# denix56/SI-Mamba

Hardware: AMD Instinct MI355X
Metric: point-clouds/sec (fwd+bwd) (higher is better)
Workload: dtype f32; 1 GPU; PointMamba classifier train step (FPS+kNN grouping, encoder, spectral SAST ordering, 12 Mamba blocks d=384 at L=1024, head, AdamW), 1024 pts -> 128 patches; global_batch=64, per_gpu_batch=64, npoints=1024, patches=128, mamba_seq_len=1024, parallelism=dp1, communicator_ranks=1, library_gemm=tuned solution table (si_mamba_amd/tuned/gemm_gfx950.csv)

## Files before the change

### include/simamba.h

```cpp
#ifndef SIMAMBA_H_
#define SIMAMBA_H_

#include <stddef.h>

#ifdef __cplusplus
extern "C" {
#endif

#define SIMAMBA_ABI_VERSION 9

#define SIMAMBA_F32  0
#define SIMAMBA_BF16 1

#define SIMAMBA_OK            0
#define SIMAMBA_E_NULLPTR    -1
#define SIMAMBA_E_SHAPE      -2
#define SIMAMBA_E_DTYPE      -3
#define SIMAMBA_E_DSTATE     -4
#define SIMAMBA_E_WIDTH      -5
#define SIMAMBA_E_WORKSPACE  -6
#define SIMAMBA_E_GROUPS     -7
#define SIMAMBA_E_ALIGN      -8
#define SIMAMBA_E_VARIANT    -9
#define SIMAMBA_E_BIAS       -10
// ... 101 lines not shown
                               void* normed, float* mean, float* rstd, int batch, int rows_per_batch,
                               int dim, float eps, int hidden_dtype, int out_dtype, void* stream);
int simamba_add_layer_norm_bwd(const void* dnormed, const float* dresidual_out,
                               const float* residual_out, const float* mean, const float* rstd,
                               const float* weight, const float* rowscale, float* dresidual,
                               void* dhidden, float* dwb_partial, int batch, int rows_per_batch,
                               int dim, int hidden_dtype, int out_dtype, void* stream);

#define SIMAMBA_NORM_RMS 1
int simamba_add_layer_norm_fwd_ex(const void* hidden, const float* residual, const float* rowscale,
                                  const float* weight, const float* bias, float* residual_out,
                                  void* normed, float* mean, float* rstd, int batch, int rows_per_batch,
                                  int dim, float eps, int hidden_dtype, int out_dtype, int flags, void* stream);
int simamba_add_layer_norm_bwd_ex(const void* dnormed, const float* dresidual_out,
                                  const float* residual_out, const float* mean, const float* rstd,
                                  const float* weight, const float* rowscale, float* dresidual,
                                  void* dhidden, float* dwb_partial, int batch, int rows_per_batch,
                                  int dim, int hidden_dtype, int out_dtype, int flags, void* stream);

int simamba_add_layer_norm_check_slots(const int* slots_host, int batch, int compact_batch);
int simamba_add_layer_norm_fwd_slots(const void* hidden, const float* residual, const float* rowscale,
                                     const float* weight, const float* bias, float* residual_out,
                                     void* normed, float* mean, float* rstd, const int* hidden_slot,
                                     int hidden_batch, const int* normed_slot, int normed_batch, int batch,
                                     int rows_per_batch, int dim, float eps, int hidden_dtype, int out_dtype,
                                     int flags, void* stream);
int simamba_add_layer_norm_bwd_slots(const void* dnormed, const float* dresidual_out,
                                     const float* residual_out, const float* mean, const float* rstd,
                                     const float* weight, const float* rowscale, float* dresidual,
                                     void* dhidden, float* dwb_partial, const int* hidden_slot,
                                     int hidden_batch, const int* normed_slot, int normed_batch, int batch,
                                     int rows_per_batch, int dim, int hidden_dtype, int out_dtype, int flags,
                                     void* stream);

int simamba_out_proj_add_ln_fwd(const void* y, const void* w, const float* residual, const float* rowscale,
                                const float* gamma, const float* beta, float* residual_out, void* normed, float* mean,
                                float* rstd, int batch, int K, int L, int C, float eps, int out_dtype, void* stream);
int simamba_out_proj_add_ln_fwd_ex(const void* y, const void* w, const float* residual, const float* rowscale,
                                   const float* gamma, const float* beta, float* residual_out, void* normed,
                                   float* mean, float* rstd, int batch, int K, int L, int C, float eps, int out_dtype,
                                   int flags, void* stream);

int simamba_in_proj_fwd(const void* x, const void* w, void* xz, int batch, int L, int C, int M, int io_dtype,
                        void* stream);

int simamba_bn_relu_grid(long long rows);
int simamba_bn_relu_fwd(const void* x, const float* gterm, int group, const float* weight, const float* bias,
                        float* running_mean, float* running_var, float momentum, float eps, int training,
                        void* y, float* mean, float* invstd, float* partial, long long rows, int C,
                        long long ld, int io_dtype, void* stream);
int simamba_bn_relu_bwd(const void* dy, const void* x, const float* gterm, int group, const float* weight,
                        const float* bias, const float* mean, const float* invstd, void* dx, float* dgterm,
                        int dgroup, float* dweight, float* dbias, float* partial, long long rows, int C,
                        long long ld, int io_dtype, int training, void* stream);
int simamba_bn_stats_local(const void* x, const float* gterm, int group, double* stats, long long stats_ld,
                           float* partial, long long rows, int C, long long ld, int io_dtype, void* stream);
int simamba_bn_stats_merge(const double* stats, int world, float* running_mean, float* running_var, float momentum,
                           float eps, float* mean, float* invstd, double* count, int C, void* stream);
int simamba_bn_relu_apply(const void* x, const float* gterm, int group, const float* weight, const float* bias,
                          const float* mean, const float* invstd, void* y, long long rows, int C, long long ld,
                          int io_dtype, void* stream);
int simamba_bn_relu_bwd_sums(const void* dy, const void* x, const float* gterm, int group, const float* weight,
                             const float* bias, const float* mean, const float* invstd, float* dweight,
                             float* dbias, float* partial, long long rows, int C, long long ld, int io_dtype,
                             void* stream);
int simamba_bn_relu_bwd_dx(const void* dy, const void* x, const float* gterm, int group, const float* weight,
// ... 156 lines not shown
```

### si_mamba_amd/_lib.py

```python
from __future__ import annotations

import ctypes
import os
from ctypes import c_char_p, c_float, c_int, c_longlong, c_size_t, c_uint, c_void_p

_HERE = os.path.dirname(os.path.abspath(__file__))
LIB_PATH = os.path.join(_HERE, "libsimamba_hip.so")

F32, BF16 = 0, 1

SPEC_SYMMETRIC = 0x01
SPEC_SELF_LOOP = 0x02
SPEC_BINARY = 0x04
SPEC_MATRIX_SYM = 0x08
SPEC_SMALLEST = 0x10
SPEC_SIGMA_MEAN = 0x20
SPEC_LARGE_G = 0x40
SPEC_MAX_G = 128
SPEC_MAX_G_LARGE = 512

SCAN_AUTO, SCAN_ROWSCAN, SCAN_LPC2, SCAN_LPC4, SCAN_MIX = 0, 1, 2, 4, 6
CKPT_ROW, CKPT_SEQ = 128, 16
BWD_DETERMINISTIC = 1
NORM_RMS = 1
# ... 38 lines not shown
    "simamba_selective_scan_dt_bwd": (c_int, [_P, _P, _P, _P, _P, _P, _P, _P, _P,
                                              _P, _P, _P, _P, _P, _P, _P, _P,
                                              c_int, c_int, c_int, c_int, c_int, c_int,
                                              _LL, _LL, _LL, _LL, _P]),
    "simamba_selective_scan_dt_bwd_ex": (c_int, [_P, _P, _P, _P, _P, _P, _P, _P, _P,
                                                 _P, _P, _P, _P, _P, _P, _P, _P,
                                                 c_int, c_int, c_int, c_int, c_int, c_int,
                                                 _LL, _LL, _LL, _LL, c_int, _P, _LL, _P]),
    "simamba_xdt_proj_fwd": (c_int, [_P, _P, _P, _P, _P, c_int, c_int, c_int, c_int, c_int, c_int, _LL, _P]),
    "simamba_conv_xdt_proj_fwd": (c_int, [_P, _P, _P, _P, _P, _P, _P, _P, c_int, c_int, c_int, c_int, c_int, c_int, _LL,
                                          _P]),
    "simamba_seq_gather_fwd": (c_int, [_P, _P, _P, c_int, c_int, c_int, c_int, _LL, c_int, _P]),
    "simamba_seq_gather_bwd": (c_int, [_P, _P, _P, c_int, c_int, c_int, c_int, c_int, _LL, c_int, _P]),
    "simamba_causal_conv1d_fwd": (c_int, [_P, _P, _P, _P, c_int, c_int, c_int, c_int, c_int, c_int, _LL, _P]),
    "simamba_causal_conv1d_bwd": (c_int, [_P, _P, _P, _P, _P, _P, _P,
                                          c_int, c_int, c_int, c_int, c_int, c_int, _LL, _LL, _P]),
    "simamba_causal_conv1d_bwd_workspace_floats": (_LL, [c_int, c_int, c_int, c_int, c_int]),
    "simamba_causal_conv1d_bwd_ex": (c_int, [_P, _P, _P, _P, _P, _P, _P,
                                             c_int, c_int, c_int, c_int, c_int, c_int, _LL, _LL, c_int, _P, _LL, _P]),
    "simamba_add_layer_norm_grid": (c_int, [c_int, c_int]),
    "simamba_add_layer_norm_fwd": (c_int, [_P, _P, _P, _P, _P, _P, _P, _P, _P, c_int, c_int, c_int, c_float,
                                           c_int, c_int, _P]),
    "simamba_add_layer_norm_bwd": (c_int, [_P, _P, _P, _P, _P, _P, _P, _P, _P, _P, c_int, c_int, c_int,
                                           c_int, c_int, _P]),
    "simamba_add_layer_norm_fwd_ex": (c_int, [_P, _P, _P, _P, _P, _P, _P, _P, _P, c_int, c_int, c_int, c_float,
                                              c_int, c_int, c_int, _P]),
    "simamba_add_layer_norm_bwd_ex": (c_int, [_P, _P, _P, _P, _P, _P, _P, _P, _P, _P, c_int, c_int, c_int,
                                              c_int, c_int, c_int, _P]),
    "simamba_add_layer_norm_check_slots": (c_int, [_P, c_int, c_int]),
    "simamba_add_layer_norm_fwd_slots": (c_int, [_P, _P, _P, _P, _P, _P, _P, _P, _P, _P, c_int, _P, c_int, c_int, c_int,
                                                 c_int, c_float, c_int, c_int, c_int, _P]),
    "simamba_add_layer_norm_bwd_slots": (c_int, [_P, _P, _P, _P, _P, _P, _P, _P, _P, _P, _P, c_int, _P, c_int, c_int,
                                                 c_int, c_int, c_int, c_int, c_int, _P]),
    "simamba_out_proj_add_ln_fwd": (c_int, [_P, _P, _P, _P, _P, _P, _P, _P, _P, _P, c_int, c_int, c_int, c_int, c_float,
                                            c_int, _P]),
    "simamba_out_proj_add_ln_fwd_ex": (c_int, [_P, _P, _P, _P, _P, _P, _P, _P, _P, _P, c_int, c_int, c_int, c_int,
                                               c_float, c_int, c_int, _P]),
    "simamba_in_proj_fwd": (c_int, [_P, _P, _P, c_int, c_int, c_int, c_int, c_int, _P]),
    "simamba_bn_relu_grid": (c_int, [_LL]),
    "simamba_bn_relu_fwd": (c_int, [_P, _P, c_int, _P, _P, _P, _P, c_float, c_float, c_int, _P, _P, _P, _P, _LL, c_int,
                                    _LL, c_int, _P]),
    "simamba_bn_relu_bwd": (c_int, [_P, _P, _P, c_int, _P, _P, _P, _P, _P, _P, c_int, _P, _P, _P, _LL, c_int, _LL,
                                    c_int, c_int, _P]),
    "simamba_bn_stats_local": (c_int, [_P, _P, c_int, _P, _LL, _P, _LL, c_int, _LL, c_int, _P]),
    "simamba_bn_stats_merge": (c_int, [_P, c_int, _P, _P, c_float, c_float, _P, _P, _P, c_int, _P]),
    "simamba_bn_relu_apply": (c_int, [_P, _P, c_int, _P, _P, _P, _P, _P, _LL, c_int, _LL, c_int, _P]),
    "simamba_bn_relu_bwd_sums": (c_int, [_P, _P, _P, c_int, _P, _P, _P, _P, _P, _P, _P, _LL, c_int, _LL, c_int, _P]),
    "simamba_bn_relu_bwd_dx": (c_int, [_P, _P, _P, c_int, _P, _P, _P, _P, _P, _P, _P, _P, _P, c_int, _LL, c_int, _LL,
                                       c_int, _P]),
    "simamba_group_max_fwd": (c_int, [_P, _P, _P, _LL, c_int, c_int, c_int, _P]),
    "simamba_group_max_bwd": (c_int, [_P, _P, _P, _LL, c_int, c_int, c_int, _P]),
    "simamba_max_linear_bwd_slabs": (c_int, [_LL, c_int]),
    "simamba_max_linear_bwd_dx": (c_int, [_P, _P, _P, _P, _LL, c_int, c_int, c_int, c_int, _P]),
    "simamba_max_linear_bwd_dw": (c_int, [_P, _P, _P, _P, _P, _LL, c_int, c_int, c_int, c_int, _P]),
    "simamba_three_nn": (c_int, [_P, _P, _P, _P, c_int, c_int, c_int, _P]),
    "simamba_three_interpolate_fwd": (c_int, [_P, _P, _P, _P, c_int, c_int, c_int, c_int, c_int, _P]),
    "simamba_three_interpolate_bwd": (c_int, [_P, _P, _P, _P, c_int, c_int, c_int, c_int, c_int, _P]),
    "simamba_gather_sum_scatter": (c_int, [_P, _P, _P, _P, c_int, c_int, c_int, c_int, c_int, c_int, _P]),
    "simamba_chamfer_fwd": (c_int, [_P, _P, _P, _P, _P, _LL, c_int, c_int, _P]),
    "simamba_chamfer_bwd": (c_int, [_P, _P, _P, _P, _P, _P, _LL, c_int, c_int, _P]),
    "simamba_chamfer_large_fwd": (c_int, [_P, _P, _P, _P, _P, _P, _P, _LL, c_int, c_int, _P]),
    "simamba_chamfer_large_bwd": (c_int, [_P, _P, _P, _P, _P, _P, _P, _LL, c_int, c_int, _P]),
    "simamba_chamfer_large_fwd_ex": (c_int, [_P, _P, _P, _P, _P, _P, _P, _LL, c_int, c_int, c_int, _P]),
    "simamba_chamfer_large_bwd_ex": (c_int, [_P, _P, _P, _P, _P, _P, _P, _LL, c_int, c_int, c_int, _P]),
    "simamba_chamfer_ragged_fwd": (c_int, [_P] * 9 + [_LL] + [c_int] * 6 + [_P]),
    "simamba_chamfer_ragged_bwd": (c_int, [_P] * 11 + [_LL] + [c_int] * 6 + [_P]),
# ... 207 lines not shown
    cell, coerce = _fuse_dt, staticmethod(_tristate)


def fuse_dt_enabled(dtype):
    import torch
    return (dtype == torch.bfloat16) if _fuse_dt[0] is None else _fuse_dt[0]


_fuse_out_norm = [True]
_hand_in_proj = [None]


class fuse_out_norm(_Override):
    cell = _fuse_out_norm


def fuse_out_norm_enabled():
    return _fuse_out_norm[0]


_drop_path_compact = [os.environ.get("SIMAMBA_DROP_PATH_COMPACT", "1").strip().lower() not in ("0", "false", "off")]
DROP_PATH_BUCKET = 4
compact_sizes = {}


class drop_path_compact(_Override):
    cell = _drop_path_compact


def drop_path_compact_enabled():
    return _drop_path_compact[0]


_sparse_max_linear = [None]


class sparse_max_linear(_Override):
    cell, coerce = _sparse_max_linear, staticmethod(_tristate)


def sparse_max_linear_enabled(dtype):
    import torch
    return (dtype == torch.float32) if _sparse_max_linear[0] is None else _sparse_max_linear[0]


class hand_in_proj(_Override):
    cell, coerce = _hand_in_proj, staticmethod(_tristate)


def in_proj_hand_enabled(workgroups, dtype=None):
    import torch
    if _hand_in_proj[0] is not None:
        return _hand_in_proj[0]
    return dtype != torch.float32 and workgroups >= IN_PROJ_MIN_WORKGROUPS


IN_PROJ_MIN_WORKGROUPS = 192


def scan_plan_step(batch, dim, seqlen, dstate, dtype, *, softplus=True, has_z=True, act_addr_or=0, a_addr=0,
                   b_addr=0, c_addr=0, z_bs=0, dz_bs=0, bc_strides=(0, 0, 0)):
    lib = load()
    code = dtype_code(dtype)
    step = _scan_ckpt[0] or lib.simamba_scan_ckpt_step(batch, dim, seqlen, dstate, code)
    if step == CKPT_SEQ and not lib.simamba_scan_seq_applicable(
            batch, dim, seqlen, dstate, code, int(bool(softplus)), int(bool(has_z)), act_addr_or, a_addr, b_addr,
# ... 66 lines not shown
```

### si_mamba_amd/block.py

```python
from __future__ import annotations

import math
from functools import partial
from typing import NamedTuple, Optional

import torch
import torch.nn as nn
from torch import Tensor

from . import _lib
from .add_norm import add_layer_norm_fn
from .cross_merge import cross_merge, cross_merge_composed, cross_merge_maps
from .mamba_simple import Mamba
from .out_norm import out_proj_add_ln_fn, out_proj_add_ln_ok
from .rms_norm import RMSNorm
from .spectral import argsort_rows, take

_KERNEL_NORMS = (nn.LayerNorm, RMSNorm)


def _fused_norm(hidden, residual, norm, rowscale=None, out_dtype=None, **compact):
    rms = type(norm) is RMSNorm
    if rms:
        _lib.count("add_rms_norm")
# ... 304 lines not shown
        y = normed = None
        if first == 0:
            l0 = self.layers[0]
            scale = l0.drop_path.rowscale(hidden_states) if isinstance(l0.drop_path, DropPath) else None
            normed, residual = _fused_norm(hidden_states, None, l0.norm, rowscale=scale)
        else:
            y = hidden_states
        n = len(self.layers)
        i = first
        while True:
            if y is not None:
                prev = self.layers[i - 1].mixer
                if i < n:
                    norm, dp = self.layers[i].norm, self.layers[i].drop_path
                    scale = dp.rowscale(y) if isinstance(dp, DropPath) else None
                    out_dtype = y.dtype
                else:
                    norm, scale, out_dtype = self.norm_f, None, self.norm_f.weight.dtype
                if out_proj_add_ln_ok(y, prev.out_proj.weight, prev.d_model):
                    rms = type(norm) is RMSNorm
                    _lib.count("out_proj_add_rms" if rms else "out_proj_add_ln")
                    normed, residual = out_proj_add_ln_fn(y, prev.out_proj.weight, residual, norm.weight, norm.bias,
                                                          norm.eps, rowscale=scale, out_dtype=out_dtype, rms=rms)
                else:
                    hidden = torch.matmul(y.transpose(1, 2), prev.out_proj.weight.t().to(y.dtype))
                    normed, residual = _fused_norm(hidden, residual, norm, rowscale=scale, out_dtype=out_dtype)
                if i == n:
                    return normed
            mixer = self.layers[i].mixer
            y = mixer.forward_xz(mixer.in_proj_xz(normed), A=A_all[i], emit_y=True)
            i += 1

    def forward(self, input_ids, pos, inference_params=None, token_index=None, balanced_index=False, *,
                route=None, drop_plan=None, drop_masks=None):
        if route is None:
            route = self.route(input_ids, token_index.shape[1] if (token_index is not None and balanced_index) else None,
                               inference_params)
        plan = drop_plan
        if plan is None:
            plan = self.draw_drop_plan(input_ids, lead=route.lead, drop_masks=drop_masks, route=route)
        elif route.stack != "compact" or plan.lead != route.lead or plan.batch != input_ids.shape[0]:
            raise ValueError("MixerModel.forward: drop_plan was drawn for another route or batch")
        if plan is not None:
            self._finish_plan(plan, input_ids.device)
            _lib.count("drop_path_compact")
        A_all = self._precompute_A()
        if route.stack == "chain" and drop_masks is not None:
            raise NotImplementedError("MixerModel.forward(drop_masks=...): the fused bf16 chain draws its own factors")
        if route.first_on_tokens:
            hidden_states, residual = self._first_block_on_distinct_tokens(
                input_ids, pos, token_index, A=A_all[0], emit_y=route.stack == "chain",
                keep=None if plan is None else (plan.sel, plan.sizes[0]))
            if plan is not None:
                residual = self._compact_ran(0, hidden_states, residual)
            hidden_states = self.drop_out_in_block(hidden_states)
            first = 1
        else:
            if token_index is not None:
                input_ids, pos = take(input_ids, token_index), take(pos, token_index)
            hidden_states, residual, first = input_ids + pos, None, 0
        if route.stack == "chain":
            return self._chain(first, hidden_states, residual, A_all)
        if plan is not None:
            return self._compact_stack(first, hidden_states, residual, A_all, plan)
        return self._layer_stack(first, hidden_states, residual, A_all, inference_params, drop_masks)

    def _layer_stack(self, first, hidden_states, residual, A_all, inference_params=None, drop_masks=None):
        for i in range(first, len(self.layers)):
            scale = drop_masks[i - 1] if (drop_masks is not None and i > 0) else None
            hidden_states, residual = self.layers[i](hidden_states, residual, inference_params=inference_params,
                                                     A=A_all[i], rowscale=scale)
            hidden_states = self.drop_out_in_block(hidden_states)
        return self._final_norm(hidden_states, residual)

    def _final_norm(self, hidden_states, residual):
        if hidden_states.is_cuda and type(self.norm_f) in _KERNEL_NORMS and hidden_states.dim() == 3:
            return _fused_norm(hidden_states, residual, self.norm_f, out_dtype=self.norm_f.weight.dtype)[0]
        residual = (hidden_states + residual) if residual is not None else hidden_states
        return self.norm_f(residual.to(dtype=self.norm_f.weight.dtype))

    def _compact_ran(self, i, hidden_states, residual):
        if hidden_states is None:
            return _SkippedMixerFn.apply(residual, *self.layers[i].mixer.parameters())
        size = hidden_states.shape[0]
        _lib.compact_sizes[size] = _lib.compact_sizes.get(size, 0) + 1
        return residual

    def _compact_stack(self, first, hidden_states, residual, A_all, plan):
        n, B = len(self.layers), plan.batch
        io = hidden_states.dtype if hidden_states is not None else self.layers[0].mixer.out_proj.weight.dtype
        for i in range(first, n):
            compact = {}
            if i > 0 and plan.sizes[i - 1] < B:
                compact.update(hidden_slot=plan.maps[i - 1], hidden_dtype=io)
            if i < n - 1 and plan.sizes[i] < B:
                compact.update(normed_slot=plan.maps[i], normed_batch=plan.sizes[i])
            hidden_states, residual = self.layers[i](hidden_states, residual, A=A_all[i],
                                                     rowscale=plan.masks[i - 1] if i > 0 else None,
                                                     draw=False, compact=compact)
            residual = self._compact_ran(i, hidden_states, residual)
            if hidden_states is not None:
                io = hidden_states.dtype
        return self._final_norm(hidden_states, residual)


class MixerModel_add(MixerModel):

    composed = False

    def forward(self, input_ids, pos, top_k_eigenvectors, N_k_top_eigenvectors, reverse, inference_params=None, *,
                order=None):
        if not reverse:
            raise ValueError("MixerModel_add: add_after_layer needs reverse=True (with reverse=False the reference "
                             "discards the merge)")
        k = int(N_k_top_eigenvectors)
        if order is None:
            vecs = top_k_eigenvectors[:, :, :k]
            B, G = vecs.shape[:2]
            order = argsort_rows(vecs.transpose(1, 2).reshape(B * k, G)).view(B, k, G)
        if order.shape[1] != k or 2 * k * order.shape[2] != input_ids.shape[1]:
            raise ValueError(f"MixerModel_add: a sequence of {input_ids.shape[1]} tokens is not 2 k G with orders "
                             f"{tuple(order.shape)} and k = {k}")
        maps = None if self.composed else cross_merge_maps(order)
        hidden_states = input_ids + pos
        residual = None
        A_all = self._precompute_A()
        for i, layer in enumerate(self.layers):
            hidden_states, residual = layer(hidden_states, residual, inference_params=inference_params, A=A_all[i])
            hidden_states = self.drop_out_in_block(hidden_states)
            hidden_states = (cross_merge_composed(hidden_states, order) if self.composed
                             else cross_merge(hidden_states, maps))
        return self._final_norm(hidden_states, residual)
```

### si_mamba_amd/point_mamba.py

```python
from __future__ import annotations

from types import SimpleNamespace

import torch
import torch.nn as nn

from . import grouping, spectral
from .block import MixerModel, MixerModel_add
from .add_norm import add_layer_norm_fn
from .encoder_ops import bn_relu_fn, group_max_fn, token_linear, token_linear_group_max


class Group(nn.Module):

    def __init__(self, num_group, group_size):
        super().__init__()
        self.num_group = num_group
        self.group_size = group_size
        self.fps_fn = grouping.sample_farthest_points

    @torch.no_grad()
    def _indices(self, xyz, lengths=None):
        if lengths is not None:
            if not (xyz.is_cuda and xyz.shape[1] <= 8192):
                raise NotImplementedError("Group: lengths are taken by the HIP kernels only (a ROCm device, clouds of "
                                          "up to 8192 points)")
            need = max(self.num_group, self.group_size)
            if not torch.cuda.is_current_stream_capturing():
                shortest = int(lengths.min())
                if shortest < need:
                    raise ValueError(f"Group: the shortest cloud has {shortest} points, every cloud needs at least "
                                     f"{need} (max of num_group = {self.num_group} and group_size = {self.group_size})")
            center, _ = self.fps_fn(xyz, self.num_group, lengths=lengths)
            return center, grouping.knn_group(center, xyz, self.group_size, lengths=lengths)
        center, _ = self.fps_fn(xyz, self.num_group)
        if xyz.is_cuda and xyz.shape[1] <= 8192:
            return center, grouping.knn_group(center, xyz, self.group_size)
        d = torch.cdist(center, xyz)
        nn_idx = d.topk(self.group_size, dim=-1, largest=False, sorted=False)[1]
        return center, nn_idx

    def forward(self, xyz, *, lengths=None):
# ... 88 lines not shown
        self.method = config.method
        self.reverse = config.reverse
        self.k_top_eigenvectors = config.k_top_eigenvectors
        self.smallest = config.smallest
        self.knn_graph = config.knn_graph
        self.symmetric = config.symmetric
        self.self_loop = config.self_loop
        self.alpha = config.alpha
        self.binary = config.binary
        self.matrix = config.matrix
        if self.method not in ("SAST", "HLT", "MAMBA"):
            raise NotImplementedError(f"ordering method {self.method!r}: SAST (:868), HLT (:1054) and MAMBA (:850) "
                                      "are built; the wavelet / RL research branches are out of scope")
        self.hlt_rand = True

    def get_loss_acc(self, ret, gt):
        loss = self.loss_ce(ret, gt.long())
        pred = ret.argmax(-1)
        acc = (pred == gt).sum() / float(gt.size(0))
        return loss, acc * 100

    def spectral_eigs(self, center):
        return spectral.spectral_order(center, self.knn_graph, self.alpha, self.k_top_eigenvectors,
                                       smallest=self.smallest, symmetric=self.symmetric,
                                       self_loop=self.self_loop, binary=self.binary, matrix=self.matrix)

    def spectral_order(self, center):
        return self.spectral_eigs(center)[2]

    def _on_tokens(self):
        return (not self.add_after_layer and self.method in ("SAST", "MAMBA")
                and not (self.training and self.drop_out.p > 0))

    def seq_len(self):
        if self.method == "MAMBA":
            return spectral.XYZ_ORDERS * self.num_group
        return spectral.sast_len(self.k_top_eigenvectors, self.num_group, self.reverse)

    def token_index(self, center, order=None):
        if self.method == "SAST":
            if order is None:
                order = self.spectral_order(center)
            return spectral.sast_index_map(order, self.reverse)
        if self.method == "MAMBA":
            return spectral.xyz_sorted_index(center)
        return None

    def order_tokens(self, tokens, pos, center, order=None):
        if self.method == "SAST" and order is None:
            order = self.spectral_order(center)
        elif self.method == "HLT":
            adj = spectral.create_graph_from_centers(center, self.knn_graph, self.alpha, self.symmetric,
                                                     self.self_loop, self.binary)
            order = spectral._eig(adj, self.k_top_eigenvectors, self.smallest, False, want_all=False)[1]
        return spectral.order_tokens(self.method, (tokens, pos), center, order, self.k_top_eigenvectors, self.reverse,
                                     self.hlt_rand)

    def forward(self, pts, gt=None, tau=None, use_wavelets=False, save_pts_dir=None, epoch=None, *, lengths=None,
                return_features=False):
        if tau is not None:
            raise NotImplementedError("PointMamba.forward(tau=...): the learned-permutation branch (reference "
                                      "models/point_mamba.py:902-952) is outside the SI-Mamba hot-path scope")
        if use_wavelets:
            raise NotImplementedError("PointMamba.forward(use_wavelets=True): the wavelet-traversal orders (reference "
                                      "models/point_mamba.py:874-880, 957-980) are outside the SI-Mamba hot-path scope; "
                                      "call with use_wavelets=False for the spectral ordering")
        want_policy = gt is not None
        if want_policy and self.method != "SAST":
            raise NotImplementedError("PointMamba.forward(gt=...): the reference defines `policy` on the SAST route only")
        on_tokens = self._on_tokens()
        route = drop_plan = None
        if on_tokens:
            like = torch.empty_strided((pts.shape[0], self.num_group, self.trans_dim), (0, 0, 0), device=pts.device)
            route = self.blocks.route(like, self.seq_len())
            drop_plan = self.blocks.draw_drop_plan(like, lead=route.lead, route=route)
        neighborhood, center, _ = self.group_divider(pts, lengths=lengths)
        join = (spectral.run_on_side_stream(lambda: self.spectral_eigs(center), center)
                if center.is_cuda and self.method == "SAST" else None)
        tokens = self.encoder(neighborhood)
        pos = self.pos_embed(center)
        spec = join() if join is not None else None
        order = None if spec is None else spec[2]
        if self.add_after_layer:
            if spec is None:
                spec = self.spectral_eigs(center)
            x, pos = self.order_tokens(tokens, pos, center, spec[2])
            x = self.drop_out(x)
            x = self.blocks(x, pos, spec[1], self.k_top_eigenvectors, self.reverse, order=spec[2])
        elif on_tokens:
            x = self.blocks(tokens, pos, token_index=self.token_index(center, order),
                            balanced_index=True,
                            route=route, drop_plan=drop_plan)
        else:
            x, pos = self.order_tokens(tokens, pos, center, order)
            x = self.drop_out(x)
            x = self.blocks(x, pos)
        if x.is_cuda and type(self.norm) is nn.LayerNorm and x.dim() == 3:
            x = add_layer_norm_fn(x, None, self.norm.weight, self.norm.bias, self.norm.eps,
                                  out_dtype=self.norm.weight.dtype)[0]
        else:
            x = self.norm(x)
        features = x.mean(1)
        ret = self.cls_head_finetune(features)
        if not want_policy:
            return (ret, features) if return_features else ret
        if spec is None:
            spec = self.spectral_eigs(center)
        vals, vecs, _ = spec
        ordered_vecs = torch.sort(vecs.transpose(1, 2), dim=-1)[0]
        policy = plackett_luce_dist(-ordered_vecs).sum(-1) + plackett_luce_dist(vals)
        return (ret, policy, features) if return_features else (ret, policy)
```

Baseline: 1172 point-clouds/s.

## Fuse final residual add, two LayerNorms and mean-pool into one kernel

Adds a HIP kernel pair that computes the last residual add, the backbone's final LayerNorm, the head LayerNorm and the token mean-pool in one pass, with a matching fused backward. The mixer stack can now return the (hidden, residual) pair so the tail can use it. The aim is to avoid writing and re-reading two full B×L×384 normalized tensors and to cut several kernel launches in both the forward and backward pass. In exchange it adds per-chunk partial buffers, an extra finish kernel and a torch sum for the parameter gradients, and it only runs for fp32 non-chain routes.

```diff
diff --git a/include/simamba.h b/include/simamba.h
--- a/include/simamba.h
+++ b/include/simamba.h
@@ -157,6 +157,15 @@
                                      int hidden_batch, const int* normed_slot, int normed_batch, int batch,
                                      int rows_per_batch, int dim, int hidden_dtype, int out_dtype, int flags,
                                      void* stream);
+
+int simamba_norm_pool_chunks(int rows_per_batch, int backward);
+int simamba_norm_pool_fwd(const float* hidden, const float* residual, const float* w1, const float* b1,
+                          const float* w2, const float* b2, float* residual_out, float* stats,
+                          float* s_partial, float* s, float* features, int batch, int rows_per_batch,
+                          int dim, float eps1, float eps2, void* stream);
+int simamba_norm_pool_bwd(const float* dfeatures, const float* residual_out, const float* stats,
+                          const float* w1, const float* b1, const float* w2, float* dx, float* dwb_partial,
+                          int batch, int rows_per_batch, int dim, void* stream);
 
 int simamba_out_proj_add_ln_fwd(const void* y, const void* w, const float* residual, const float* rowscale,
                                 const float* gamma, const float* beta, float* residual_out, void* normed, float* mean,
diff --git a/si_mamba_amd/_lib.py b/si_mamba_amd/_lib.py
--- a/si_mamba_amd/_lib.py
+++ b/si_mamba_amd/_lib.py
@@ -94,6 +94,9 @@
                                                  c_int, c_float, c_int, c_int, c_int, _P]),
     "simamba_add_layer_norm_bwd_slots": (c_int, [_P, _P, _P, _P, _P, _P, _P, _P, _P, _P, _P, c_int, _P, c_int, c_int,
                                                  c_int, c_int, c_int, c_int, c_int, _P]),
+    "simamba_norm_pool_chunks": (c_int, [c_int, c_int]),
+    "simamba_norm_pool_fwd": (c_int, [_P] * 11 + [c_int, c_int, c_int, c_float, c_float, _P]),
+    "simamba_norm_pool_bwd": (c_int, [_P] * 8 + [c_int, c_int, c_int, _P]),
     "simamba_out_proj_add_ln_fwd": (c_int, [_P, _P, _P, _P, _P, _P, _P, _P, _P, _P, c_int, c_int, c_int, c_int, c_float,
                                             c_int, _P]),
     "simamba_out_proj_add_ln_fwd_ex": (c_int, [_P, _P, _P, _P, _P, _P, _P, _P, _P, _P, c_int, c_int, c_int, c_int,
@@ -367,6 +370,21 @@
     return _drop_path_compact[0]
 
 
+def _env_on(name):
+    return os.environ.get(name, "1").strip().lower() not in ("0", "false", "off")
+
+
+_fused_tail = [_env_on("SIMAMBA_FUSED_TAIL")]
+
+
+class fused_tail(_Override):
+    cell = _fused_tail
+
+
+def fused_tail_enabled():
+    return _fused_tail[0]
+
+
 _sparse_max_linear = [None]
 
 
diff --git a/si_mamba_amd/block.py b/si_mamba_amd/block.py
--- a/si_mamba_amd/block.py
+++ b/si_mamba_amd/block.py
@@ -360,7 +360,7 @@
             i += 1
 
     def forward(self, input_ids, pos, inference_params=None, token_index=None, balanced_index=False, *,
-                route=None, drop_plan=None, drop_masks=None):
+                route=None, drop_plan=None, drop_masks=None, return_pair=False):
         if route is None:
             route = self.route(input_ids, token_index.shape[1] if (token_index is not None and balanced_index) else None,
                                inference_params)
@@ -388,17 +388,22 @@
                 input_ids, pos = take(input_ids, token_index), take(pos, token_index)
             hidden_states, residual, first = input_ids + pos, None, 0
         if route.stack == "chain":
+            if return_pair:
+                raise ValueError("MixerModel.forward(return_pair=True): the fused bf16 chain ends in its final norm")
             return self._chain(first, hidden_states, residual, A_all)
         if plan is not None:
-            return self._compact_stack(first, hidden_states, residual, A_all, plan)
-        return self._layer_stack(first, hidden_states, residual, A_all, inference_params, drop_masks)
-
-    def _layer_stack(self, first, hidden_states, residual, A_all, inference_params=None, drop_masks=None):
+            return self._compact_stack(first, hidden_states, residual, A_all, plan, return_pair)
+        return self._layer_stack(first, hidden_states, residual, A_all, inference_params, drop_masks, return_pair)
+
+    def _layer_stack(self, first, hidden_states, residual, A_all, inference_params=None, drop_masks=None,
+                     return_pair=False):
         for i in range(first, len(self.layers)):
             scale = drop_masks[i - 1] if (drop_masks is not None and i > 0) else None
             hidden_states, residual = self.layers[i](hidden_states, residual, inference_params=inference_params,
                                                      A=A_all[i], rowscale=scale)
             hidden_states = self.drop_out_in_block(hidden_states)
+        if return_pair:
+            return hidden_states, residual
         return self._final_norm(hidden_states, residual)
 
     def _final_norm(self, hidden_states, residual):
@@ -414,7 +419,7 @@
         _lib.compact_sizes[size] = _lib.compact_sizes.get(size, 0) + 1
         return residual
 
-    def _compact_stack(self, first, hidden_states, residual, A_all, plan):
+    def _compact_stack(self, first, hidden_states, residual, A_all, plan, return_pair=False):
         n, B = len(self.layers), plan.batch
         io = hidden_states.dtype if hidden_states is not None else self.layers[0].mixer.out_proj.weight.dtype
         for i in range(first, n):
@@ -429,6 +434,8 @@
             residual = self._compact_ran(i, hidden_states, residual)
             if hidden_states is not None:
                 io = hidden_states.dtype
+        if return_pair:
+            return hidden_states, residual
         return self._final_norm(hidden_states, residual)
 
 
diff --git a/si_mamba_amd/csrc/norm_pool.hip b/si_mamba_amd/csrc/norm_pool.hip
--- /dev/null
+++ b/si_mamba_amd/csrc/norm_pool.hip
@@ -0,0 +1,321 @@
+#include "common.h"
+
+namespace simamba {
+
+constexpr int kPoolThreads = 256;
+constexpr int kPoolWaves = kPoolThreads / 64;
+constexpr int kPoolMaxChunks = 2;
+constexpr int kPoolRowsFwd = 32;
+constexpr int kPoolRowsBwd = 64;
+
+struct PoolArgs {
+  const float* hidden;
+  const float* residual;
+  const float* w1;
+  const float* b1;
+  const float* w2;
+  const float* b2;
+  float* residual_out;
+  float* stats;
+  float* s_partial;
+  float* s;
+  float* features;
+  const float* dfeatures;
+  float* dx;
+  float* dwb_partial;
+  int batch, rows_per_batch, dim, chunks;
+  float eps1, eps2;
+};
+
+__device__ __forceinline__ float sum4(float4 v) { return (v.x + v.y) + (v.z + v.w); }
+
+__device__ __forceinline__ void pool_combine(const float* sred, int stride, int count, float* out) {
+  for (int i = threadIdx.x; i < count; i += kPoolThreads) {
+    float v = 0.f;
+#pragma unroll
+    for (int wv = 0; wv < kPoolWaves; ++wv) v += sred[wv * stride + i];
+    out[i] = v;
+  }
+}
+
+template <int kChunks>
+__global__ __launch_bounds__(kPoolThreads) void norm_pool_fwd_kernel(PoolArgs p) {
+  extern __shared__ float sred[];
+  const int lane = threadIdx.x & 63;
+  const int wave = threadIdx.x >> 6;
+  const int b = blockIdx.x / p.chunks;
+  const int ch = blockIdx.x - b * p.chunks;
+  const int r0 = ch * kPoolRowsFwd;
+  const int r1 = min(r0 + kPoolRowsFwd, p.rows_per_batch);
+  const int nch = p.dim >> 2;
+  float4 w1[kChunks], b1[kChunks], acc[kChunks];
+#pragma unroll
+  for (int k = 0; k < kChunks; ++k) {
+    const int c = lane + 64 * k;
+    w1[k] = c < nch ? *reinterpret_cast<const float4*>(p.w1 + 4 * c) : make_float4(0, 0, 0, 0);
+    b1[k] = c < nch ? *reinterpret_cast<const float4*>(p.b1 + 4 * c) : make_float4(0, 0, 0, 0);
+    acc[k] = make_float4(0, 0, 0, 0);
+  }
+  const float inv_dim = 1.f / p.dim;
+  for (int r = r0 + wave; r < r1; r += kPoolWaves) {
+    const size_t row = static_cast<size_t>(b) * p.rows_per_batch + r;
+    const size_t base = row * p.dim;
+    float4 x[kChunks];
+    float sum = 0.f;
+#pragma unroll
+    for (int k = 0; k < kChunks; ++k) {
+      const int c = lane + 64 * k;
+      if (c < nch) {
+        float4 h = *reinterpret_cast<const float4*>(p.hidden + base + 4 * c);
+        const float4 rr = *reinterpret_cast<const float4*>(p.residual + base + 4 * c);
+        h.x += rr.x; h.y += rr.y; h.z += rr.z; h.w += rr.w;
+        *reinterpret_cast<float4*>(p.residual_out + base + 4 * c) = h;
+        x[k] = h;
+        sum += sum4(h);
+      } else {
+        x[k] = make_float4(0, 0, 0, 0);
+      }
+    }
+    const float mu1 = wave_allreduce_sum(sum) * inv_dim;
+    float sq = 0.f;
+#pragma unroll
+    for (int k = 0; k < kChunks; ++k) {
+      if (lane + 64 * k < nch) {
+        x[k].x -= mu1; x[k].y -= mu1; x[k].z -= mu1; x[k].w -= mu1;
+        sq += (x[k].x * x[k].x + x[k].y * x[k].y) + (x[k].z * x[k].z + x[k].w * x[k].w);
+      }
+    }
+    const float rs1 = rsqrtf(wave_allreduce_sum(sq) * inv_dim + p.eps1);
+    sum = 0.f;
+#pragma unroll
+    for (int k = 0; k < kChunks; ++k) {
+      if (lane + 64 * k < nch) {
+        x[k].x = fmaf(x[k].x * rs1, w1[k].x, b1[k].x);
+        x[k].y = fmaf(x[k].y * rs1, w1[k].y, b1[k].y);
+        x[k].z = fmaf(x[k].z * rs1, w1[k].z, b1[k].z);
+        x[k].w = fmaf(x[k].w * rs1, w1[k].w, b1[k].w);
+        sum += sum4(x[k]);
+      }
+    }
+    const float mu2 = wave_allreduce_sum(sum) * inv_dim;
+    sq = 0.f;
+#pragma unroll
+    for (int k = 0; k < kChunks; ++k) {
+      if (lane + 64 * k < nch) {
+        x[k].x -= mu2; x[k].y -= mu2; x[k].z -= mu2; x[k].w -= mu2;
+        sq += (x[k].x * x[k].x + x[k].y * x[k].y) + (x[k].z * x[k].z + x[k].w * x[k].w);
+      }
+    }
+    const float rs2 = rsqrtf(wave_allreduce_sum(sq) * inv_dim + p.eps2);
+#pragma unroll
+    for (int k = 0; k < kChunks; ++k) {
+      acc[k].x = fmaf(x[k].x, rs2, acc[k].x); acc[k].y = fmaf(x[k].y, rs2, acc[k].y);
+      acc[k].z = fmaf(x[k].z, rs2, acc[k].z); acc[k].w = fmaf(x[k].w, rs2, acc[k].w);
+    }
+    if (lane == 0) *reinterpret_cast<float4*>(p.stats + 4 * row) = make_float4(mu1, rs1, mu2, rs2);
+  }
+  float* mine = sred + wave * p.dim;
+#pragma unroll
+  for (int k = 0; k < kChunks; ++k) {
+    const int c = lane + 64 * k;
+    if (c < nch) *reinterpret_cast<float4*>(mine + 4 * c) = acc[k];
+  }
+  __syncthreads();
+  pool_combine(sred, p.dim, p.dim, p.s_partial + static_cast<size_t>(blockIdx.x) * p.dim);
+}
+
+__global__ __launch_bounds__(kPoolThreads) void norm_pool_finish_kernel(PoolArgs p) {
+  const long long i = static_cast<long long>(blockIdx.x) * kPoolThreads + threadIdx.x;
+  if (i >= static_cast<long long>(p.batch) * p.dim) return;
+  const int b = static_cast<int>(i / p.dim), c = static_cast<int>(i - static_cast<long long>(b) * p.dim);
+  const float* part = p.s_partial + static_cast<size_t>(b) * p.chunks * p.dim + c;
+  float acc = 0.f;
+  int k = 0;
+  for (; k + 8 <= p.chunks; k += 8) {
+    float v[8];
+#pragma unroll
+    for (int m = 0; m < 8; ++m) v[m] = part[static_cast<size_t>(k + m) * p.dim];
+#pragma unroll
+    for (int m = 0; m < 8; ++m) acc += v[m];
+  }
+  for (; k < p.chunks; ++k) acc += part[static_cast<size_t>(k) * p.dim];
+  p.s[i] = acc;
+  p.features[i] = fmaf(p.w2[c], acc * (1.f / p.rows_per_batch), p.b2[c]);
+}
+
+template <int kChunks>
+__global__ __launch_bounds__(kPoolThreads) void norm_pool_bwd_kernel(PoolArgs p) {
+  extern __shared__ float sred[];
+  const int lane = threadIdx.x & 63;
+  const int wave = threadIdx.x >> 6;
+  const int b = blockIdx.x / p.chunks;
+  const int ch = blockIdx.x - b * p.chunks;
+  const int r0 = ch * kPoolRowsBwd;
+  const int r1 = min(r0 + kPoolRowsBwd, p.rows_per_batch);
+  const int nch = p.dim >> 2;
+  const float inv_dim = 1.f / p.dim;
+  const float inv_rows = 1.f / p.rows_per_batch;
+  float4 w1[kChunks], b1[kChunks], g2[kChunks], dw[kChunks], db[kChunks];
+  float sg2 = 0.f;
+#pragma unroll
+  for (int k = 0; k < kChunks; ++k) {
+    const int c = lane + 64 * k;
+    w1[k] = b1[k] = g2[k] = dw[k] = db[k] = make_float4(0, 0, 0, 0);
+    if (c < nch) {
+      w1[k] = *reinterpret_cast<const float4*>(p.w1 + 4 * c);
+      b1[k] = *reinterpret_cast<const float4*>(p.b1 + 4 * c);
+      const float4 df = *reinterpret_cast<const float4*>(p.dfeatures + static_cast<size_t>(b) * p.dim + 4 * c);
+      const float4 w2 = *reinterpret_cast<const float4*>(p.w2 + 4 * c);
+      g2[k] = make_float4(df.x * inv_rows * w2.x, df.y * inv_rows * w2.y, df.z * inv_rows * w2.z,
+                          df.w * inv_rows * w2.w);
+      sg2 += sum4(g2[k]);
+    }
+  }
+  const float mg2 = wave_allreduce_sum(sg2) * inv_dim;
+  for (int r = r0 + wave; r < r1; r += kPoolWaves) {
+    const size_t row = static_cast<size_t>(b) * p.rows_per_batch + r;
+    const size_t base = row * p.dim;
+    const float4 st = *reinterpret_cast<const float4*>(p.stats + 4 * row);
+    float4 xh1[kChunks], xh2[kChunks];
+    float s2 = 0.f;
+#pragma unroll
+    for (int k = 0; k < kChunks; ++k) {
+      const int c = lane + 64 * k;
+      xh1[k] = xh2[k] = make_float4(0, 0, 0, 0);
+      if (c < nch) {
+        const float4 x = *reinterpret_cast<const float4*>(p.residual_out + base + 4 * c);
+        xh1[k] = make_float4((x.x - st.x) * st.y, (x.y - st.x) * st.y, (x.z - st.x) * st.y, (x.w - st.x) * st.y);
+        xh2[k].x = (fmaf(xh1[k].x, w1[k].x, b1[k].x) - st.z) * st.w;
+        xh2[k].y = (fmaf(xh1[k].y, w1[k].y, b1[k].y) - st.z) * st.w;
+        xh2[k].z = (fmaf(xh1[k].z, w1[k].z, b1[k].z) - st.z) * st.w;
+        xh2[k].w = (fmaf(xh1[k].w, w1[k].w, b1[k].w) - st.z) * st.w;
+        s2 += (g2[k].x * xh2[k].x + g2[k].y * xh2[k].y) + (g2[k].z * xh2[k].z + g2[k].w * xh2[k].w);
+      }
+    }
+    const float c2 = wave_allreduce_sum(s2) * inv_dim;
+    float t1 = 0.f, t2 = 0.f;
+    float4 g1[kChunks];
+#pragma unroll
+    for (int k = 0; k < kChunks; ++k) {
+      g1[k] = make_float4(0, 0, 0, 0);
+      if (lane + 64 * k < nch) {
+        float4 dn;
+        dn.x = (g2[k].x - mg2 - xh2[k].x * c2) * st.w;
+        dn.y = (g2[k].y - mg2 - xh2[k].y * c2) * st.w;
+        dn.z = (g2[k].z - mg2 - xh2[k].z * c2) * st.w;
+        dn.w = (g2[k].w - mg2 - xh2[k].w * c2) * st.w;
+        dw[k].x = fmaf(dn.x, xh1[k].x, dw[k].x); dw[k].y = fmaf(dn.y, xh1[k].y, dw[k].y);
+        dw[k].z = fmaf(dn.z, xh1[k].z, dw[k].z); dw[k].w = fmaf(dn.w, xh1[k].w, dw[k].w);
+        db[k].x += dn.x; db[k].y += dn.y; db[k].z += dn.z; db[k].w += dn.w;
+        g1[k] = make_float4(dn.x * w1[k].x, dn.y * w1[k].y, dn.z * w1[k].z, dn.w * w1[k].w);
+        t1 += sum4(g1[k]);
+        t2 += (g1[k].x * xh1[k].x + g1[k].y * xh1[k].y) + (g1[k].z * xh1[k].z + g1[k].w * xh1[k].w);
+      }
+    }
+    const float c1 = wave_allreduce_sum(t1) * inv_dim;
+    const float c3 = wave_allreduce_sum(t2) * inv_dim;
+#pragma unroll
+    for (int k = 0; k < kChunks; ++k) {
+      const int c = lane + 64 * k;
+      if (c < nch) {
+        float4 dx;
+        dx.x = (g1[k].x - c1 - xh1[k].x * c3) * st.y;
+        dx.y = (g1[k].y - c1 - xh1[k].y * c3) * st.y;
+        dx.z = (g1[k].z - c1 - xh1[k].z * c3) * st.y;
+        dx.w = (g1[k].w - c1 - xh1[k].w * c3) * st.y;
+        *reinterpret_cast<float4*>(p.dx + base + 4 * c) = dx;
+      }
+    }
+  }
+  float* mine = sred + wave * 2 * p.dim;
+#pragma unroll
+  for (int k = 0; k < kChunks; ++k) {
+    const int c = lane + 64 * k;
+    if (c < nch) {
+      *reinterpret_cast<float4*>(mine + 4 * c) = dw[k];
+      *reinterpret_cast<float4*>(mine + p.dim + 4 * c) = db[k];
+    }
+  }
+  __syncthreads();
+  pool_combine(sred, 2 * p.dim, 2 * p.dim, p.dwb_partial + static_cast<size_t>(blockIdx.x) * 2 * p.dim);
+}
+
+static int pool_chunks(int rows_per_batch, int rows_per_wg) { return (rows_per_batch + rows_per_wg - 1) / rows_per_wg; }
+
+}
+
+using namespace simamba;
+
+static int check_pool(int batch, int rows_per_batch, int dim) {
+  if (batch < 0 || rows_per_batch < 0) return SIMAMBA_E_SHAPE;
+  if (dim <= 0 || (dim & 3) || dim > 64 * 4 * kPoolMaxChunks) return SIMAMBA_E_SHAPE;
+  if (static_cast<long long>(batch) * rows_per_batch > 0x7fffffffll) return SIMAMBA_E_SHAPE;
+  return SIMAMBA_OK;
+}
+
+extern "C" int simamba_norm_pool_chunks(int rows_per_batch, int backward) {
+  if (rows_per_batch < 0) return SIMAMBA_E_SHAPE;
+  return pool_chunks(rows_per_batch, backward ? kPoolRowsBwd : kPoolRowsFwd);
+}
+
+extern "C" int simamba_norm_pool_fwd(const float* hidden, const float* residual, const float* w1, const float* b1,
+                                     const float* w2, const float* b2, float* residual_out, float* stats,
+                                     float* s_partial, float* s, float* features, int batch, int rows_per_batch,
+                                     int dim, float eps1, float eps2, void* stream) {
+  const int rc = check_pool(batch, rows_per_batch, dim);
+  if (rc) return rc;
+  if (batch == 0) return SIMAMBA_OK;
+  if (rows_per_batch == 0) return SIMAMBA_E_SHAPE;
+  if (!hidden || !residual || !w1 || !b1 || !w2 || !b2 || !residual_out || !stats || !s_partial || !s || !features)
+    return SIMAMBA_E_NULLPTR;
+  const uintptr_t bits = reinterpret_cast<uintptr_t>(hidden) | reinterpret_cast<uintptr_t>(residual) |
+                         reinterpret_cast<uintptr_t>(w1) | reinterpret_cast<uintptr_t>(b1) |
+                         reinterpret_cast<uintptr_t>(residual_out) | reinterpret_cast<uintptr_t>(stats);
+  if (bits & 15u) return SIMAMBA_E_ALIGN;
+  PoolArgs a{};
+  a.hidden = hidden; a.residual = residual; a.w1 = w1; a.b1 = b1; a.w2 = w2; a.b2 = b2;
+  a.residual_out = residual_out; a.stats = stats; a.s_partial = s_partial; a.s = s; a.features = features;
+  a.batch = batch; a.rows_per_batch = rows_per_batch; a.dim = dim; a.eps1 = eps1; a.eps2 = eps2;
+  a.chunks = pool_chunks(rows_per_batch, kPoolRowsFwd);
+  hipStream_t st = static_cast<hipStream_t>(stream);
+  const int grid = batch * a.chunks;
+  const size_t lds = sizeof(float) * kPoolWaves * dim;
+  if (dim <= 256)
+    hipLaunchKernelGGL(norm_pool_fwd_kernel<1>, dim3(grid), dim3(kPoolThreads), lds, st, a);
+  else
+    hipLaunchKernelGGL(norm_pool_fwd_kernel<2>, dim3(grid), dim3(kPoolThreads), lds, st, a);
+  int err = static_cast<int>(hipGetLastError());
+  if (err) return err;
+  const long long outs = static_cast<long long>(batch) * dim;
+  hipLaunchKernelGGL(norm_pool_finish_kernel, dim3(static_cast<unsigned>((outs + kPoolThreads - 1) / kPoolThreads)),
+                     dim3(kPoolThreads), 0, st, a);
+  return static_cast<int>(hipGetLastError());
+}
+
+extern "C" int simamba_norm_pool_bwd(const float* dfeatures, const float* residual_out, const float* stats,
+                                     const float* w1, const float* b1, const float* w2, float* dx, float* dwb_partial,
+                                     int batch, int rows_per_batch, int dim, void* stream) {
+  const int rc = check_pool(batch, rows_per_batch, dim);
+  if (rc) return rc;
+  if (batch == 0) return SIMAMBA_OK;
+  if (rows_per_batch == 0) return SIMAMBA_E_SHAPE;
+  if (!dfeatures || !residual_out || !stats || !w1 || !b1 || !w2 || !dx || !dwb_partial) return SIMAMBA_E_NULLPTR;
+  const uintptr_t bits = reinterpret_cast<uintptr_t>(dfeatures) | reinterpret_cast<uintptr_t>(residual_out) |
+                         reinterpret_cast<uintptr_t>(stats) | reinterpret_cast<uintptr_t>(w1) |
+                         reinterpret_cast<uintptr_t>(b1) | reinterpret_cast<uintptr_t>(w2) |
+                         reinterpret_cast<uintptr_t>(dx);
+  if (bits & 15u) return SIMAMBA_E_ALIGN;
+  PoolArgs a{};
+  a.dfeatures = dfeatures; a.residual_out = const_cast<float*>(residual_out); a.stats = const_cast<float*>(stats);
+  a.w1 = w1; a.b1 = b1; a.w2 = w2; a.dx = dx; a.dwb_partial = dwb_partial;
+  a.batch = batch; a.rows_per_batch = rows_per_batch; a.dim = dim;
+  a.chunks = pool_chunks(rows_per_batch, kPoolRowsBwd);
+  const int grid = batch * a.chunks;
+  const size_t lds = sizeof(float) * kPoolWaves * 2 * dim;
+  hipStream_t st = static_cast<hipStream_t>(stream);
+  if (dim <= 256)
+    hipLaunchKernelGGL(norm_pool_bwd_kernel<1>, dim3(grid), dim3(kPoolThreads), lds, st, a);
+  else
+    hipLaunchKernelGGL(norm_pool_bwd_kernel<2>, dim3(grid), dim3(kPoolThreads), lds, st, a);
+  return static_cast<int>(hipGetLastError());
+}
diff --git a/si_mamba_amd/norm_pool.py b/si_mamba_amd/norm_pool.py
--- /dev/null
+++ b/si_mamba_amd/norm_pool.py
@@ -0,0 +1,74 @@
+from __future__ import annotations
+
+import torch
+
+from . import _lib
+
+MAX_DIM = 512
+
+
+def norm_pool_ok(hidden, residual, norm1, norm2):
+    nn = torch.nn
+    if not (residual is not None and hidden is not None and hidden.is_cuda and hidden.dim() == 3
+            and hidden.dtype == torch.float32 and residual.dtype == torch.float32 and residual.shape == hidden.shape
+            and not torch.is_autocast_enabled("cuda")):
+        return False
+    dim = hidden.shape[-1]
+    if dim % 4 or dim > MAX_DIM or hidden.shape[1] == 0:
+        return False
+    for n in (norm1, norm2):
+        if not (type(n) is nn.LayerNorm and n.elementwise_affine and n.bias is not None
+                and tuple(n.normalized_shape) == (dim,) and n.weight.dtype == torch.float32):
+            return False
+    return True
+
+
+def _aligned(t):
+    return t if t.data_ptr() % 16 == 0 else t.clone()
+
+
+class NormPoolFn(torch.autograd.Function):
+    @staticmethod
+    def forward(ctx, hidden, residual, w1, b1, eps1, w2, b2, eps2):
+        _lib.require_gpu(hidden, "norm_pool_fn")
+        if hidden.dtype != torch.float32 or residual.dtype != torch.float32:
+            raise TypeError("norm_pool_fn: fp32 hidden and residual only")
+        if hidden.dim() != 3 or residual.shape != hidden.shape:
+            raise ValueError(f"norm_pool_fn: hidden {tuple(hidden.shape)} against residual {tuple(residual.shape)}")
+        h, r = _aligned(hidden.contiguous()), _aligned(residual.contiguous())
+        Bsz, L, dim = h.shape
+        dev = h.device
+        f32 = dict(device=dev, dtype=torch.float32)
+        w1c, b1c, w2c, b2c = (t.float().contiguous() for t in (w1, b1, w2, b2))
+        chunks = _lib.load().simamba_norm_pool_chunks(L, 0)
+        res_out = torch.empty(Bsz, L, dim, **f32)
+        stats = torch.empty(Bsz * L, 4, **f32)
+        s_part = torch.empty(Bsz, chunks, dim, **f32)
+        s = torch.empty(Bsz, dim, **f32)
+        features = torch.empty(Bsz, dim, **f32)
+        _lib.call("simamba_norm_pool_fwd", h, r, w1c, b1c, w2c, b2c, res_out, stats, s_part, s, features, Bsz, L, dim,
+                  float(eps1), float(eps2), device=dev, time_as="norm_pool_fwd")
+        ctx.save_for_backward(res_out, stats, s, w1c, b1c, w2c)
+        ctx.param_dtypes = (w1.dtype, b1.dtype, w2.dtype, b2.dtype)
+        return features
+
+    @staticmethod
+    def backward(ctx, dfeatures):
+        res_out, stats, s, w1c, b1c, w2c = ctx.saved_tensors
+        Bsz, L, dim = res_out.shape
+        dev = res_out.device
+        df = _aligned(dfeatures.float().contiguous())
+        chunks = _lib.load().simamba_norm_pool_chunks(L, 1)
+        dx = torch.empty_like(res_out)
+        part = torch.empty(Bsz * chunks, 2, dim, device=dev, dtype=torch.float32)
+        _lib.call("simamba_norm_pool_bwd", df, res_out, stats, w1c, b1c, w2c, dx, part, Bsz, L, dim, device=dev,
+                  time_as="norm_pool_bwd")
+        dwb1 = part.sum(0)
+        dw2 = (df * s).sum(0) / L
+        db2 = df.sum(0)
+        t1, t2, t3, t4 = ctx.param_dtypes
+        return dx, dx, dwb1[0].to(t1), dwb1[1].to(t2), None, dw2.to(t3), db2.to(t4), None
+
+
+def norm_pool_fn(hidden, residual, w1, b1, eps1, w2, b2, eps2):
+    return NormPoolFn.apply(hidden, residual, w1, b1, eps1, w2, b2, eps2)
diff --git a/si_mamba_amd/point_mamba.py b/si_mamba_amd/point_mamba.py
--- a/si_mamba_amd/point_mamba.py
+++ b/si_mamba_amd/point_mamba.py
@@ -5,9 +5,10 @@
 import torch
 import torch.nn as nn
 
-from . import grouping, spectral
+from . import _lib, grouping, spectral
 from .block import MixerModel, MixerModel_add
 from .add_norm import add_layer_norm_fn
+from .norm_pool import norm_pool_fn, norm_pool_ok
 from .encoder_ops import bn_relu_fn, group_max_fn, token_linear, token_linear_group_max
 
 
@@ -162,6 +163,18 @@
         return (not self.add_after_layer and self.method in ("SAST", "MAMBA")
                 and not (self.training and self.drop_out.p > 0))
 
+    def _fused_tail_applies(self, pts, route, return_features=False):
+        if not (_lib.fused_tail_enabled() and pts.is_cuda and not self.add_after_layer
+                and not (return_features and not self.training)
+                and not torch.is_autocast_enabled("cuda")
+                and type(self.norm) is nn.LayerNorm and type(self.blocks.norm_f) is nn.LayerNorm
+                and self.norm.weight.dtype == torch.float32 and self.blocks.norm_f.weight.dtype == torch.float32):
+            return False
+        if route is None:
+            like = torch.empty_strided((pts.shape[0], self.num_group, self.trans_dim), (0, 0, 0), device=pts.device)
+            route = self.blocks.route(like, None)
+        return route.stack != "chain"
+
     def seq_len(self):
         if self.method == "MAMBA":
             return spectral.XYZ_ORDERS * self.num_group
@@ -211,6 +224,7 @@
         pos = self.pos_embed(center)
         spec = join() if join is not None else None
         order = None if spec is None else spec[2]
+        fuse_tail = self._fused_tail_applies(pts, route, return_features)
         if self.add_after_layer:
             if spec is None:
                 spec = self.spectral_eigs(center)
@@ -220,17 +234,25 @@
         elif on_tokens:
             x = self.blocks(tokens, pos, token_index=self.token_index(center, order),
                             balanced_index=True,
-                            route=route, drop_plan=drop_plan)
+                            route=route, drop_plan=drop_plan, return_pair=fuse_tail)
         else:
             x, pos = self.order_tokens(tokens, pos, center, order)
             x = self.drop_out(x)
-            x = self.blocks(x, pos)
-        if x.is_cuda and type(self.norm) is nn.LayerNorm and x.dim() == 3:
-            x = add_layer_norm_fn(x, None, self.norm.weight, self.norm.bias, self.norm.eps,
-                                  out_dtype=self.norm.weight.dtype)[0]
+            x = self.blocks(x, pos, return_pair=fuse_tail)
+        norm_f = self.blocks.norm_f
+        if fuse_tail and norm_pool_ok(x[0], x[1], norm_f, self.norm):
+            _lib.count("fused_tail")
+            features = norm_pool_fn(x[0], x[1], norm_f.weight, norm_f.bias, norm_f.eps, self.norm.weight,
+                                    self.norm.bias, self.norm.eps)
         else:
-            x = self.norm(x)
-        features = x.mean(1)
+            if fuse_tail:
+                x = self.blocks._final_norm(*x)
+            if x.is_cuda and type(self.norm) is nn.LayerNorm and x.dim() == 3:
+                x = add_layer_norm_fn(x, None, self.norm.weight, self.norm.bias, self.norm.eps,
+                                      out_dtype=self.norm.weight.dtype)[0]
+            else:
+                x = self.norm(x)
+            features = x.mean(1)
         ret = self.cls_head_finetune(features)
         if not want_policy:
             return (ret, features) if return_features else ret
```

Result: no change. 1177 point-clouds/s (median of 6 runs) (+0.5%).
